# lhotse-speech/lhotse

Measured on AMD Instinct MI355X. Metric: cuts/sec (10 s @16 kHz -> 80-dim log-mel fbank), higher is better.
Workload: dtype f32

## Files before the change

### lhotse_amd/csrc/fft_common.hpp

```cpp
#pragma once
#include "common.hpp"

namespace hipfeat {

typedef float v2 __attribute__((ext_vector_type(2)));
typedef float f32x4 __attribute__((ext_vector_type(4)));

template <int CTRL>
__device__ __forceinline__ float dpp_mov(float v) {
  return __builtin_bit_cast(float, __builtin_amdgcn_update_dpp(0, __builtin_bit_cast(int, v), CTRL, 0xF, 0xF, true));
}
__device__ __forceinline__ float dpp_shr1_keep(float keep, float v) {
  return __builtin_bit_cast(float, __builtin_amdgcn_update_dpp(__builtin_bit_cast(int, keep), __builtin_bit_cast(int, v), 0x111, 0xF, 0xF, false));
}
constexpr int DPP_QUAD(int a, int b, int c, int d) { return a | (b << 2) | (c << 4) | (d << 6); }
constexpr int DPP_ROW_SHR1 = 0x111;
constexpr int DPP_ROW_ROR1 = 0x121;
constexpr int DPP_ROW_MIRROR = 0x140;
constexpr int DPP_ROW_HALF_MIRROR = 0x141;

__device__ __forceinline__ float row16_sum(float v) {
  v += dpp_mov<DPP_QUAD(1, 0, 3, 2)>(v);
  v += dpp_mov<DPP_QUAD(2, 3, 0, 1)>(v);
  v += dpp_mov<DPP_ROW_HALF_MIRROR>(v);
// ... 75 lines not shown
    const v2 d = hi ? x[n] - x[n + 16] : x[n];
    if (n == 0) o[n] = d;
    else if (n == 8) o[n] = rot_mi(d);
    else o[n] = cmulc(d, v2{C[n], -S[n]}, v2{S[n], C[n]});
  }
  fft16(e, E);
  fft16(o, O);
#pragma unroll
  for (int k = 0; k < 16; ++k) {
    X[2 * k] = E[k];
    X[2 * k + 1] = O[k];
  }
}

__device__ __forceinline__ void fft8(const v2* x, v2* X) {
  constexpr float R2 = 0.70710678118654752f;
  v2 e[4], o[4];
  {
    const v2 s0 = x[0] + x[4], s1 = x[0] - x[4], s2 = x[2] + x[6], u3 = swap2(x[2] - x[6]);
    e[0] = s0 + s2, e[2] = s0 - s2, e[1] = u3 * HF_CJ + s1, e[3] = u3 * HF_NCJ + s1;
  }
  {
    const v2 s0 = x[1] + x[5], s1 = x[1] - x[5], s2 = x[3] + x[7], u3 = swap2(x[3] - x[7]);
    o[0] = s0 + s2, o[2] = s0 - s2, o[1] = u3 * HF_CJ + s1, o[3] = u3 * HF_NCJ + s1;
  }
  o[1] = cmulc(o[1], v2{R2, -R2}, v2{R2, R2});
  o[2] = rot_mi(o[2]);
  o[3] = cmulc(o[3], v2{-R2, -R2}, v2{R2, -R2});
#pragma unroll
  for (int k = 0; k < 4; ++k) {
    X[k] = e[k] + o[k];
    X[k + 4] = e[k] - o[k];
  }
}

__device__ __forceinline__ void mel4_reduce_floor(const f32x4 acc, float m4, float m8, float floor_, float (&v)[4]) {
  float v0 = acc[0], v1 = acc[1], v2_ = acc[2], v3 = acc[3];
  asm volatile(
      "s_nop 7\n\t"
      "v_fmac_f32_dpp %0, %0, %4 row_shr:4 row_mask:0xf bank_mask:0xf bound_ctrl:1\n\t"
      "v_fmac_f32_dpp %1, %1, %4 row_shr:4 row_mask:0xf bank_mask:0xf bound_ctrl:1\n\t"
      "v_fmac_f32_dpp %2, %2, %4 row_shr:4 row_mask:0xf bank_mask:0xf bound_ctrl:1\n\t"
      "v_fmac_f32_dpp %3, %3, %4 row_shr:4 row_mask:0xf bank_mask:0xf bound_ctrl:1\n\t"
      "v_fmac_f32_dpp %0, %0, %5 row_shr:8 row_mask:0xf bank_mask:0xf bound_ctrl:1\n\t"
      "v_fmac_f32_dpp %1, %1, %5 row_shr:8 row_mask:0xf bank_mask:0xf bound_ctrl:1\n\t"
      "v_fmac_f32_dpp %2, %2, %5 row_shr:8 row_mask:0xf bank_mask:0xf bound_ctrl:1\n\t"
      "v_fmac_f32_dpp %3, %3, %5 row_shr:8 row_mask:0xf bank_mask:0xf bound_ctrl:1\n\t"
      "v_max_f32 %0, %0, %6\n\tv_max_f32 %1, %1, %6\n\tv_max_f32 %2, %2, %6\n\tv_max_f32 %3, %3, %6"
      : "+v"(v0), "+v"(v1), "+v"(v2_), "+v"(v3)
      : "v"(m4), "v"(m8), "v"(floor_));
  v[0] = v0, v[1] = v1, v[2] = v2_, v[3] = v3;
}
template <int ROWS>
__device__ __forceinline__ void mel4_store(float* o, int64_t stride, int nf, const float* v) {
  if (nf >= ROWS) {
#pragma unroll
    for (int i = 0; i < ROWS; ++i) o[i * stride] = v[i];
  } else {
#pragma unroll
    for (int i = 0; i < ROWS - 1; ++i)
      if (i < nf) o[i * stride] = v[i];
  }
}
template <int ROWS>
__device__ __forceinline__ void mel4_store_saddr(float* row0, unsigned col, int64_t stride, int nf, const float* v) {
  const unsigned off = col * 4u;
#pragma unroll
  for (int i = 0; i < ROWS; ++i) {
    if (i < nf) {
      const float* base = row0 + i * stride;
      asm volatile("global_store_dword %0, %1, %2" : : "v"(off), "v"(v[i]), "s"(base) : "memory");
    }
  }
}

__device__ __forceinline__ float fast_log(float x) {
#ifdef HIPFEAT_ACCURATE_LOG
  return logf(x);
#else
  return __builtin_amdgcn_logf(x) * 0.69314718055994531f;
#endif
}

}
```

### lhotse_amd/csrc/hipfeat.hip

```cpp
#include "../../include/hipfeat.h"

#include <hip/hip_runtime.h>

#include <algorithm>
#include <atomic>
#include <cmath>
#include <cstdarg>
#include <cstdio>
#include <cstring>
#include <map>
#include <mutex>
#include <new>
#include <string>
#include <vector>

#include "common.hpp"
#include "kernel_generic.hpp"
#include "fft512_common.hpp"
#include "kernel_fft512b.hpp"
#include "kernel_fft512c.hpp"
#include "kernel_fft1024c.hpp"
#include "kernel_fft2048c.hpp"
#include "plan_tables.hpp"
#include "kernel_resample.hpp"
// ... 5 lines not shown
#include "kernel_level.hpp"
#include "kernel_sinc.hpp"
#include "kernel_specaug.hpp"
#include "kernel_whisper2.hpp"
#include "kernel_whisper3.hpp"
#include "layout_rounds.hpp"
#include "kernel_fft256.hpp"
#include "kernel_fft256c.hpp"
#include "kernel_wave.hpp"
#include "host_bulk.hpp"

using namespace hipfeat;

static thread_local char g_err[512] = "";

static inline const char* route_env(const char* name) { return getenv(name); }
#ifdef HIPFEAT_EXPERIMENTS
static inline const char* exp_env(const char* name) { return getenv(name); }
#else
static inline const char* exp_env(const char*) { return nullptr; }
#endif

static hipfeat_status fail(hipfeat_status st, const char* fmt, ...) {
  va_list ap;
  va_start(ap, fmt);
  vsnprintf(g_err, sizeof(g_err), fmt, ap);
  va_end(ap);
  return st;
}

#define HIP_TRY(expr)                                                                          \
  do {                                                                                         \
    hipError_t e_ = (expr);                                                                    \
    if (e_ != hipSuccess)                                                                      \
      return fail(HIPFEAT_ERR_HIP, "%s failed: %s (%s:%d)", #expr, hipGetErrorName(e_), __FILE__, __LINE__); \
  } while (0)

struct DeviceGuard {
  int prev = -1;
  bool ok = true;
  explicit DeviceGuard(int dev) {
    if (hipGetDevice(&prev) != hipSuccess) prev = -1;
    if (prev != dev) ok = (hipSetDevice(dev) == hipSuccess);
  }
  ~DeviceGuard() {
    int cur = -1;
    if (prev >= 0 && hipGetDevice(&cur) == hipSuccess && cur != prev) (void)hipSetDevice(prev);
  }
};

struct StagingSlot {
  void* h = nullptr;
  void* d = nullptr;
  size_t cap = 0;
  hipEvent_t ev = nullptr;
  bool busy = false;
};

enum class Route {
  Generic,
  Fft512b,
  Fft256b,
  Wave,
  Whisper2,
  Fft512c,
  Fft1024c,
  Whisper3,
  Fft2048c,
  Fft256c,
};

struct hipfeat_plan {
  hipfeat_config cfg{};
  int device = 0;
  int feature_dim = 0;
  int K = 0, H = 0, log2H = 0;
  bool pow2 = false;
  int npad_left = 0;
  std::string kernel_name = "generic";
  int blocks_per_cu = 0;
  Route route = Route::Generic;
  const void* fn = nullptr;
  const void* fn_flat = nullptr;
  int block = 0;
  size_t lds = 0;
  float* d_window = nullptr;
  float2* d_tw = nullptr;
  float* d_mel = nullptr;
  int2* d_mel_range = nullptr;
  float* d_dct = nullptr;
  float* d_lifter = nullptr;
  int fpb = 8;
  int span = 0, off_z = 0, off_p = 0, off_tw = 0, off_stat = 0, off_mel = 0;
  float* d_mel_a4 = nullptr;
  float* d_dct_consts = nullptr;
  int lm_stride = 0, dct_groups = 0, dct_floats = 0;
  int tiles_per_block = 4;
  int xs_floats = 0;
  int const_floats = 0;
  float* d_lds_consts = nullptr;
  float* d_mel_a = nullptr;
  WaveWork* d_work = nullptr;
  float* d_c_shared = nullptr;
  int c_shared_floats = 0, c_wtab_off = 0, c_ltab_off = 0, c_xs_floats = 0;
  int fpb_unit = 0, c_rounds_max = 0;
  int w_nsets = 0, w_steps[kWMaxSets] = {}, w_step0[kWMaxSets] = {};
  float* d_x_twp = nullptr;
  int x_waves = 0, x_tws_off = 0, x_tw32_off = 0;
  float* d_mel_t = nullptr;
  int wave_blob_floats = 0;
  bool wave_dct_in_lds = false;
  float* d_wh2_cs = nullptr;
  float* d_wh2_tw = nullptr;
  float* d_wh2_mel = nullptr;
  int32_t* d_wh2_sched = nullptr;
  mutable std::mutex mu;
  mutable StagingSlot slots[4];
  mutable int next_slot = 0;
  mutable float* d_scratch_wave = nullptr;
  mutable size_t scratch_wave_cap = 0;
  mutable float* d_scratch_out = nullptr;
  mutable size_t scratch_out_cap = 0;
};

struct hipfeat_layout {
  int device = 0;
  int64_t batch = 0;
  int64_t total_frames = 0;
  int64_t total_blocks = 0;
  int64_t out_row_stride = 0;
  int uniform_bpc = 0;
  int fpb = 0, fpb_unit = 0;
  CutDesc* d_cuts = nullptr;
  bool owns = true;
  std::vector<int64_t> num_frames;
  std::vector<int32_t> block_cut;
  bool flat = false;
  int64_t total_quads = 0;
  unsigned char* d_norm = nullptr;
  int norm_slots = 0;
  mutable std::atomic<unsigned> norm_next{0};
};
constexpr int kNormSlots = 4;
static size_t norm_slot_bytes(const hipfeat_layout* lay) { return (2 * (size_t)lay->total_blocks + (size_t)lay->batch) * 4; }

extern "C" HIPFEAT_API int32_t hipfeat_abi_version(void) { return HIPFEAT_ABI_VERSION; }
extern "C" HIPFEAT_API const char* hipfeat_last_error(void) { return g_err; }

extern "C" HIPFEAT_API hipfeat_status hipfeat_device_count(int32_t* count) {
  if (!count) return fail(HIPFEAT_ERR_INVALID, "count is NULL");
  int n = 0;
  hipError_t e = hipGetDeviceCount(&n);
  if (e != hipSuccess) {
    *count = 0;
    return fail(HIPFEAT_ERR_HIP, "hipGetDeviceCount failed: %s", hipGetErrorName(e));
  }
  *count = n;
  return HIPFEAT_OK;
}

extern "C" HIPFEAT_API int64_t hipfeat_num_frames(int64_t num_samples, int32_t frame_length, int32_t frame_shift,
                                      int32_t snip_edges) {
  if (frame_shift <= 0 || frame_length <= 0 || num_samples < 0) return 0;
  if (snip_edges) return num_samples < frame_length ? 0 : 1 + (num_samples - frame_length) / frame_shift;
  return (num_samples + frame_shift / 2) / frame_shift;
}
// ... 66 lines not shown
}

#ifdef HIPFEAT_LDS_POISON
static void set_lds_poison(size_t bytes) {
  const int n = (int)(bytes / sizeof(float));
  (void)hipMemcpyToSymbol(HIP_SYMBOL(hipfeat::g_lds_poison_floats), &n, sizeof(n));
}
#else
static inline void set_lds_poison(size_t) {}
#endif

static hipError_t ensure_dynamic_lds(const void* fn, size_t bytes) {
  static std::mutex mu;
  static std::map<std::pair<const void*, int>, size_t> high;
  int dev = 0;
  (void)hipGetDevice(&dev);
  std::lock_guard<std::mutex> lk(mu);
  size_t& cur = high[{fn, dev}];
  if (bytes <= cur) return hipSuccess;
  hipError_t e = hipFuncSetAttribute(fn, hipFuncAttributeMaxDynamicSharedMemorySize, (int)bytes);
  if (e == hipSuccess) cur = bytes;
  return e;
}

static hipfeat_status claim(hipfeat_plan* p, Route route, const void* fn, int block, size_t lds) {
  hipError_t e = ensure_dynamic_lds(fn, lds);
  if (e != hipSuccess) return fail(HIPFEAT_ERR_HIP, "hipFuncSetAttribute(dynamic LDS = %zu B) failed: %s", lds, hipGetErrorName(e));
  int nb = 0;
  if (hipOccupancyMaxActiveBlocksPerMultiprocessor(&nb, fn, block, lds) == hipSuccess) p->blocks_per_cu = nb;
  p->route = route;
  p->fn = fn;
  p->block = block;
  p->lds = lds;
  return HIPFEAT_OK;
}

static hipfeat_status claim_wave_auto(hipfeat_plan* p, Route route, const void* fn, const WaveAutoTables& t, int frames, int rounds, int rounds_max,
                                      const std::string& head) {
  hipfeat_status st;
  if ((st = upload(&p->d_c_shared, t.image.data(), t.image.size())) != HIPFEAT_OK) return st;
  if (!t.dct.empty() && (st = upload(&p->d_dct_consts, t.dct.data(), t.dct.size())) != HIPFEAT_OK) return st;
  if (!t.twp.empty() && (st = upload(&p->d_x_twp, t.twp.data(), t.twp.size())) != HIPFEAT_OK) return st;
  p->c_shared_floats = t.shared_floats;
  p->c_wtab_off = t.wtab_off;
  p->c_ltab_off = t.ltab_off;
  p->c_xs_floats = t.xs_floats;
  p->x_tws_off = t.tws_off;
  p->x_tw32_off = t.tw32_off;
  p->w_nsets = t.w_nsets;
  std::copy(t.w_steps, t.w_steps + 4, p->w_steps);
  std::copy(t.w_step0, t.w_step0 + 4, p->w_step0);
  p->fpb_unit = t.waves * frames;
  p->fpb = p->fpb_unit * rounds;
  p->c_rounds_max = rounds_max;
  if ((st = claim(p, route, fn, 64 * t.waves, t.lds)) != HIPFEAT_OK) return st;
  p->kernel_name = head + strf(" lds=%zuB blocks/CU=%d mel4=%dx%d", t.lds, p->blocks_per_cu, t.sch_nsets, t.sch_steps);
  return HIPFEAT_OK;
}

static hipfeat_status claim_tile(hipfeat_plan* p, Route route, const void* fn, const TileTables& t, int tile_frames, const char* kernel) {
  const hipfeat_config& c = p->cfg;
  const bool mfcc = c.kind == HIPFEAT_MFCC, spec = c.kind == HIPFEAT_SPECTROGRAM || c.kind == HIPFEAT_LOG_SPECTROGRAM;
  hipfeat_status st;
  if ((st = upload(&p->d_lds_consts, t.consts.data(), t.consts.size())) != HIPFEAT_OK) return st;
  if (route == Route::Fft512b && (st = upload(&p->d_mel_a, t.mel_a.data(), t.mel_a.size())) != HIPFEAT_OK) return st;
  if ((st = upload(&p->d_work, t.work, 4)) != HIPFEAT_OK) return st;
  if ((st = upload(&p->d_mel_a4, t.mel_a4.data(), t.mel_a4.size())) != HIPFEAT_OK) return st;
  if (mfcc && (st = upload(&p->d_dct_consts, t.dct.data(), t.dct.size())) != HIPFEAT_OK) return st;
  p->tiles_per_block = 16;
  p->fpb = tile_frames * p->tiles_per_block;
  p->const_floats = (int)t.consts.size();
  p->xs_floats = t.xs_floats;
  p->lm_stride = t.lm_stride;
  p->dct_groups = t.dct_groups;
  p->dct_floats = (int)t.dct.size();
  if ((st = claim(p, route, fn, 256, t.lds)) != HIPFEAT_OK) return st;
  p->kernel_name = strf("%s<%d,%d> %s lds=%zuB blocks/CU=%d", kernel, t.nrows, mfcc ? 1 : (spec ? 2 : 0), mfcc ? "mfcc" : (spec ? "spectrogram" : "fbank"), t.lds,
                        p->blocks_per_cu);
  return HIPFEAT_OK;
}

static bool fft512c_has_flat(int nrows, int N) { return nrows == 13 && N >= 384; }

template <int MODE>
static const void* fft512c_pick(int nrows, int N, bool flat) {
  if (flat && fft512c_has_flat(nrows, N)) return entry<fft512c_kernel<13, 12, MODE, true>>();
  if (nrows == 10) return entry<fft512c_kernel<10, 0, MODE>>();
  if (nrows == 13 && N >= 384) return entry<fft512c_kernel<13, 12, MODE>>();
  if (nrows == 13) return entry<fft512c_kernel<13, 0, MODE>>();
  return entry<fft512c_kernel<16, 0, MODE>>();
}
static const void* fft512c_dispatch(int mode, int nrows, int N, bool flat) {
  return mode == 0 ? fft512c_pick<0>(nrows, N, flat)
                   : (mode == 1 ? fft512c_pick<1>(nrows, N, flat) : (mode == 2 ? fft512c_pick<2>(nrows, N, flat) : fft512c_pick<3>(nrows, N, flat)));
}

static hipfeat_status setup_fft512c(hipfeat_plan* p, const PlanInputs& in, int nrows) {
  const bool mfcc = p->cfg.kind == HIPFEAT_MFCC;
  if (mfcc && (in.M > 4 * kCDctChunks || in.C > 64 || !in.dct)) return HIPFEAT_OK;
  const WaveAutoTables t = build_fft512c_tables(in, nrows, {kCPRowStride, kCMaxSets, kCMaxSteps, kCWaves, kCRegion}, kCDctChunks, kCDctChunksSmall);
  if (!t.fits || t.lds > 80 * 1024 || (t.xs_floats >> 8) > 6) return HIPFEAT_OK;
  hipfeat_status st = claim_wave_auto(p, Route::Fft512c, fft512c_dispatch(t.mode, nrows, in.N, false), t, 4, 8, 16,
                                      strf("fft512c_kernel<%d> %s", nrows, mfcc ? "mfcc" : "fbank"));
  if (st == HIPFEAT_OK && fft512c_has_flat(nrows, in.N)) {
    p->fn_flat = fft512c_dispatch(t.mode, nrows, in.N, true);
    hipError_t e = ensure_dynamic_lds(p->fn_flat, t.lds);
    if (e != hipSuccess) return fail(HIPFEAT_ERR_HIP, "hipFuncSetAttribute(dynamic LDS = %zu B) failed: %s", t.lds, hipGetErrorName(e));
  }
  return st;
}

static hipfeat_status setup_fft512(hipfeat_plan* p, const PlanInputs& in) {
  const hipfeat_config& c = p->cfg;
  const char* force = route_env("HIPFEAT_FORCE_GENERIC");
  if (force && force[0] == '1') return HIPFEAT_OK;
  const bool mfcc = c.kind == HIPFEAT_MFCC;
  const bool spec = c.kind == HIPFEAT_SPECTROGRAM || c.kind == HIPFEAT_LOG_SPECTROGRAM;
  if (c.kind > HIPFEAT_MFCC || c.fft_length != 512 || (in.shift & 1) || in.N < 32 || c.use_energy || (!spec && c.use_fft_mag))
    return HIPFEAT_OK;
  if (mfcc && (in.M > 8 * kMaxDctGroups || in.C > 64)) return HIPFEAT_OK;
  const int need = (in.N + 31) / 32;
  const int nrows = need <= 10 ? 10 : (need <= 13 ? 13 : 16);
  if ((in.M + 15) / 16 > 8) return HIPFEAT_OK;

  if (!spec) {
    const char* var = route_env("HIPFEAT_FFT512_VARIANT");
    if (!(var && var[0] == 'b')) {
      hipfeat_status stc = setup_fft512c(p, in, nrows);
      if (stc != HIPFEAT_OK || p->route == Route::Fft512c) return stc;
    }
  }
  const TileTables t = build_tile_tables(in, nrows, {16, kPRowStride, kMaxGroups0, kMaxGroups1, kTileFrames, kBWaveRegion, false});
  if (!t.fits || t.lds > 160 * 1024) return HIPFEAT_OK;
  const void* fn;
  if (mfcc)
    fn = nrows == 10 ? entry<fft512b_kernel<10, 1>>() : (nrows == 13 ? entry<fft512b_kernel<13, 1>>() : entry<fft512b_kernel<16, 1>>());
  else if (spec)
    fn = nrows == 10 ? entry<fft512b_kernel<10, 2>>() : (nrows == 13 ? entry<fft512b_kernel<13, 2>>() : entry<fft512b_kernel<16, 2>>());
  else
    fn = nrows == 10 ? entry<fft512b_kernel<10, 0>>() : (nrows == 13 ? entry<fft512b_kernel<13, 0>>() : entry<fft512b_kernel<16, 0>>());
  return claim_tile(p, Route::Fft512b, fn, t, kTileFrames, "fft512b_kernel");
}

static hipfeat_status setup_fft1024c(hipfeat_plan* p, const PlanInputs& in) {
  const hipfeat_config& c = p->cfg;
  const int N = in.N, shift = in.shift;
  const bool librosa = c.kind == HIPFEAT_LIBROSA_FBANK;
  if ((c.kind != HIPFEAT_FBANK && !librosa) || c.fft_length != 1024 || (shift & 1) || N < 32 * 17 || c.use_energy ||
      (c.use_fft_mag && !librosa) || route_env("HIPFEAT_FORCE_GENERIC") || route_env("HIPFEAT_NO_WAVE_AUTONOMOUS"))
    return HIPFEAT_OK;
  const int need = (N + 31) / 32;
  const int nrows = need <= 20 ? 20 : (need <= 26 ? 26 : 32);
  static const int kFixedSteps[5][3] = {{0, 0, 0}, {24, 16, 8}, {24, 16, 8}, {24, 24, 8}, {16, 16, 8}};
  int want = 0;
  if (route_env("HIPFEAT_NO_FIXED_SCHEDULE")) want = 0;
  else if (nrows == 32) want = !c.remove_dc_offset && c.preemph_coeff == 0.0f ? 4 : 0;
  else if (!librosa && !c.use_fft_mag && in.M == 80 && !c.snip_edges)
    want = N == 600 && shift == 240 ? 1 : (N == 800 && shift == 320 ? 2 : (N == 551 && shift == 220 ? 3 : 0));
  const WaveAutoTables t = build_fft1024c_tables(in, nrows, {kWPRowStride, kWMaxSets, kWMaxSteps, kWWaves, kWRegion}, kWSplitSteps, kWWavesFixed, want ? kFixedSteps[want] : nullptr);
  if (!t.fits || t.lds > 160 * 1024 || (t.xs_floats >> 8) > 10) return HIPFEAT_OK;
  const int fixed = t.fixed ? want : 0;
  const void* fn = fixed == 1 ? entry<fft1024c_kernel<20, 24, 16, 8>>()
                   : fixed == 2 ? entry<fft1024c_kernel<26, 24, 16, 8>>()
                   : fixed == 3 ? entry<fft1024c_kernel<20, 24, 24, 8>>()
                   : fixed == 4 ? entry<fft1024c_kernel<32, 16, 16, 8, true>>()
                   : nrows == 20 ? entry<fft1024c_kernel<20>>() : (nrows == 26 ? entry<fft1024c_kernel<26>>() : entry<fft1024c_kernel<32>>());
  return claim_wave_auto(p, Route::Fft1024c, fn, t, 4, 8, 32, strf("fft1024c_kernel<%d> fbank%s waves=%d", nrows, fixed ? " fixed-schedule" : "", t.waves));
}

static hipfeat_status setup_fft256c(hipfeat_plan* p, const PlanInputs& in, int nrows) {
  const WaveAutoTables t = build_fft256c_tables(in, nrows, {kDPRowStride, kDSets, kDSteps, kDWaves, kDRegion});
  if (!t.fits || t.lds > 80 * 1024 || (t.xs_floats >> 8) > 6) return HIPFEAT_OK;
  const void* fn = nrows == 13 ? (in.N >= 192 ? entry<fft256c_kernel<13, 12>>() : entry<fft256c_kernel<13, 0>>()) : entry<fft256c_kernel<16, 0>>();
  return claim_wave_auto(p, Route::Fft256c, fn, t, 8, 4, 16, strf("fft256c_kernel<%d> fbank", nrows));
}

static hipfeat_status setup_fft256(hipfeat_plan* p, const PlanInputs& in) {
  const hipfeat_config& c = p->cfg;
  const bool mfcc = c.kind == HIPFEAT_MFCC;
  const bool spec = c.kind == HIPFEAT_SPECTROGRAM || c.kind == HIPFEAT_LOG_SPECTROGRAM;
  if (c.kind > HIPFEAT_MFCC || c.fft_length != 256 || (in.shift & 1) || in.N < 16 || c.use_energy || (!spec && c.use_fft_mag) ||
      route_env("HIPFEAT_FORCE_GENERIC"))
    return HIPFEAT_OK;
  if (mfcc && (in.M > 8 * kMaxDctGroups || in.C > 64)) return HIPFEAT_OK;
  const int nrows = (in.N + 15) / 16 <= 13 ? 13 : 16;
  if ((in.M + 15) / 16 > 8) return HIPFEAT_OK;
  if (!mfcc && !spec) {
    const char* var = route_env("HIPFEAT_FFT256_VARIANT");
    if (!(var && var[0] == 'b') && !route_env("HIPFEAT_NO_WAVE_AUTONOMOUS")) {
// ... 516 lines not shown
      w2.out = d_out;
      w2.cuts = lay->d_cuts;
      w2.window = plan->d_window;
      w2.cs = plan->d_wh2_cs;
      w2.tw = plan->d_wh2_tw;
      w2.mel_a = plan->d_wh2_mel;
      w2.out_stride = lay->out_row_stride;
      w2.num_cuts = (int32_t)lay->batch;
      w2.uniform_bpc = lay->uniform_bpc;
      w2.M = c.num_filters;
      w2.mel_floor = c.mel_floor;
      w2.sched = plan->d_wh2_sched;
      arg = &w2;
      break;
    case Route::Whisper3:
      fill_wave_autonomous(w3, plan, lay, d_wave, d_out);
      w3.cs = plan->d_wh2_cs;
      w3.total_blocks = (int32_t)lay->total_blocks;
      if (lay->d_norm) {
        unsigned char* slot = lay->d_norm + (size_t)(lay->norm_next.fetch_add(1u) % (unsigned)lay->norm_slots) * norm_slot_bytes(lay);
        w3.wg_stat = reinterpret_cast<float*>(slot);
        w3.cut_done = reinterpret_cast<uint32_t*>(slot + 2 * (size_t)lay->total_blocks * sizeof(float));
      }
      arg = &w3;
      break;
    case Route::Fft512c:
      cp.dct_tab = plan->d_dct_consts;
      cp.C = c.num_ceps;
      cp.total_quads = (int32_t)lay->total_quads;
      [[fallthrough]];
    case Route::Fft256c:
      fill_wave_autonomous(cp, plan, lay, d_wave, d_out);
      fill_frames(cp, plan);
      arg = &cp;
      break;
    case Route::Fft1024c:
      fill_wave_autonomous(kp, plan, lay, d_wave, d_out);
      fill_frames(kp, plan);
      kp.nsets = plan->w_nsets;
      for (int s2 = 0; s2 < kWMaxSets; ++s2) kp.steps[s2] = plan->w_steps[s2], kp.step0[s2] = plan->w_step0[s2];
      arg = &kp;
      break;
    case Route::Fft2048c:
      fill_wave_autonomous(xp, plan, lay, d_wave, d_out);
      fill_frames(xp, plan);
      xp.twp = plan->d_x_twp;
      xp.waves = plan->x_waves;
      xp.tws_off = plan->x_tws_off;
      xp.tw32_off = plan->x_tw32_off;
      xp.nsets = plan->w_nsets;
      for (int s2 = 0; s2 < kXMaxSets; ++s2) xp.steps[s2] = plan->w_steps[s2], xp.step0[s2] = plan->w_step0[s2];
      arg = &xp;
      break;
    case Route::Fft512b:
    case Route::Fft256b:
      bp.wave = d_wave;
      bp.out = d_out;
      bp.cuts = lay->d_cuts;
      bp.lds_consts = plan->d_lds_consts;
      bp.mel_a = plan->d_mel_a4;
      bp.work = plan->d_work;
      bp.out_stride = lay->out_row_stride;
      bp.num_cuts = (int32_t)lay->batch;
      bp.uniform_bpc = lay->uniform_bpc;
      bp.tiles_per_block = plan->tiles_per_block;
      bp.N = c.frame_length;
      bp.shift = c.frame_shift;
      bp.npad_left = plan->npad_left;
      bp.M = c.num_filters;
      bp.flags = (c.remove_dc_offset ? F_REMOVE_DC : 0) | (c.use_fft_mag ? F_FFT_MAG : 0) | (c.kind == HIPFEAT_LOG_SPECTROGRAM ? F_LOG_SPEC : 0);
      bp.log_offset = c.log_offset;
      bp.preemph = c.preemph_coeff;
      bp.mel_floor = c.mel_floor;
      bp.xs_floats = plan->xs_floats;
      bp.const_floats = plan->const_floats;
      bp.dct_consts = plan->d_dct_consts;
      bp.C = c.num_ceps;
      bp.lm_stride = plan->lm_stride;
      bp.dct_groups = plan->dct_groups;
      bp.dct_floats = plan->dct_floats;
      arg = &bp;
      break;
  }
  const void* fn = lay->flat && plan->fn_flat ? plan->fn_flat : plan->fn;
  void* args[] = {arg};
  DeviceGuard g(plan->device);
  set_lds_poison(plan->lds);
  (void)hipLaunchKernel(fn, dim3((unsigned)lay->total_blocks), dim3(plan->block), args, plan->lds, stream);
  HIP_TRY(hipGetLastError());
  if (whisper && !(plan->route == Route::Whisper3 && lay->d_norm)) {
    hipLaunchKernelGGL(whisper_norm_kernel, dim3((unsigned)lay->batch), dim3(1024), 0, stream, lay->d_cuts, d_out, lay->out_row_stride,
                       (int32_t)c.num_filters, (int32_t)c.frame_shift);
    HIP_TRY(hipGetLastError());
  }
  return HIPFEAT_OK;
}

extern "C" HIPFEAT_API hipfeat_status hipfeat_extract_layout(const hipfeat_plan* plan, const hipfeat_layout* layout,
                                                 const float* d_wave, float* d_out, void* stream) {
  if (!plan || !layout) return fail(HIPFEAT_ERR_INVALID, "plan/layout is NULL");
  return launch(plan, layout, d_wave, d_out, (hipStream_t)stream);
}

__global__ __launch_bounds__(256) void fill_padding_kernel(const CutDesc* __restrict__ cuts, float* __restrict__ out, int64_t row_stride,
                                                           int32_t rows_per_cut, int32_t feature_dim, float value) {
  const CutDesc cd = cuts[blockIdx.y];
  const int64_t n = (int64_t)(rows_per_cut - cd.num_frames) * feature_dim;
  float* __restrict__ base = out + (cd.out_row + cd.num_frames) * row_stride;
  for (int64_t i = (int64_t)blockIdx.x * 256 + threadIdx.x; i < n; i += (int64_t)gridDim.x * 256) {
    const int64_t r = i / feature_dim;
    base[r * row_stride + (i - r * feature_dim)] = value;
  }
}

__global__ __launch_bounds__(256) void pcm16_to_float_kernel(const int16_t* __restrict__ in, float* __restrict__ out, int64_t n) {
  const int64_t n8 = n >> 3;
  const bool aligned = ((reinterpret_cast<uintptr_t>(in) & 15) == 0) && ((reinterpret_cast<uintptr_t>(out) & 15) == 0);
  constexpr float k = 1.0f / 32768.0f;
  if (aligned) {
    for (int64_t i = (int64_t)blockIdx.x * 256 + threadIdx.x; i < n8; i += (int64_t)gridDim.x * 256) {
      const int4 v = reinterpret_cast<const int4*>(in)[i];
      const int w[4] = {v.x, v.y, v.z, v.w};
      float4 a, b;
      a.x = (float)(int16_t)(w[0] & 0xffff) * k; a.y = (float)(w[0] >> 16) * k;
      a.z = (float)(int16_t)(w[1] & 0xffff) * k; a.w = (float)(w[1] >> 16) * k;
      b.x = (float)(int16_t)(w[2] & 0xffff) * k; b.y = (float)(w[2] >> 16) * k;
      b.z = (float)(int16_t)(w[3] & 0xffff) * k; b.w = (float)(w[3] >> 16) * k;
      reinterpret_cast<float4*>(out)[2 * i] = a;
      reinterpret_cast<float4*>(out)[2 * i + 1] = b;
    }
    for (int64_t i = (n8 << 3) + (int64_t)blockIdx.x * 256 + threadIdx.x; i < n; i += (int64_t)gridDim.x * 256) out[i] = (float)in[i] * k;
  } else {
    for (int64_t i = (int64_t)blockIdx.x * 256 + threadIdx.x; i < n; i += (int64_t)gridDim.x * 256) out[i] = (float)in[i] * k;
  }
}

extern "C" HIPFEAT_API hipfeat_status hipfeat_pcm16_to_float(const int16_t* d_pcm, float* d_wave, int64_t num_samples, void* stream) {
  if (num_samples < 0 || (num_samples > 0 && (!d_pcm || !d_wave))) return fail(HIPFEAT_ERR_INVALID, "bad pcm16 arguments");
  if (num_samples == 0) return HIPFEAT_OK;
  const int64_t blocks = std::min<int64_t>((num_samples / 8 + 255) / 256 + 1, 256 * 32);
  hipLaunchKernelGGL(pcm16_to_float_kernel, dim3((unsigned)blocks), dim3(256), 0, (hipStream_t)stream, d_pcm, d_wave, num_samples);
  hipError_t e = hipGetLastError();
  if (e != hipSuccess) return fail(HIPFEAT_ERR_HIP, "pcm16 launch failed: %s", hipGetErrorName(e));
  return HIPFEAT_OK;
}

__global__ __launch_bounds__(256) void float_to_half_kernel(const float* __restrict__ in, uint16_t* __restrict__ out, int64_t n) {
  const int64_t n8 = n >> 3;
  const bool aligned = ((reinterpret_cast<uintptr_t>(in) & 15) == 0) && ((reinterpret_cast<uintptr_t>(out) & 15) == 0);
  auto cvt = [](float x) -> unsigned { return (unsigned)__builtin_bit_cast(unsigned short, (_Float16)x); };
  if (aligned) {
    for (int64_t i = (int64_t)blockIdx.x * 256 + threadIdx.x; i < n8; i += (int64_t)gridDim.x * 256) {
      const float4 a = reinterpret_cast<const float4*>(in)[2 * i], b = reinterpret_cast<const float4*>(in)[2 * i + 1];
      uint4 o;
      o.x = cvt(a.x) | (cvt(a.y) << 16);
      o.y = cvt(a.z) | (cvt(a.w) << 16);
      o.z = cvt(b.x) | (cvt(b.y) << 16);
      o.w = cvt(b.z) | (cvt(b.w) << 16);
      reinterpret_cast<uint4*>(out)[i] = o;
    }
    for (int64_t i = (n8 << 3) + (int64_t)blockIdx.x * 256 + threadIdx.x; i < n; i += (int64_t)gridDim.x * 256) out[i] = (uint16_t)cvt(in[i]);
  } else {
    for (int64_t i = (int64_t)blockIdx.x * 256 + threadIdx.x; i < n; i += (int64_t)gridDim.x * 256) out[i] = (uint16_t)cvt(in[i]);
  }
}

extern "C" HIPFEAT_API hipfeat_status hipfeat_float_to_half(const float* d_in, uint16_t* d_out, int64_t n, void* stream) {
// ... 1698 lines not shown
```

### lhotse_amd/csrc/kernel_fft512c.hpp

```cpp
#pragma once
#include "common.hpp"
#include "fft_common.hpp"

namespace hipfeat {

constexpr int kCExRowStride = 34;
constexpr int kCExFrameStride = 8 * kCExRowStride + 16;
constexpr int kCPRowStride = 272;
constexpr int kCRegion = 4 * kCExFrameStride + 16;
constexpr int kCMaxSets = 2;
constexpr int kCMaxSteps = 16;
constexpr int kCWaves = 8;
constexpr int kCLmStride = 48;
constexpr int kCDctChunks = 10;
constexpr int kCDctChunksSmall = 6;

struct Fft512cParams {
  const float* wave;
  float* out;
  const CutDesc* cuts;
  const float* shared_consts;
  int64_t out_stride;
  int32_t num_cuts, uniform_bpc;
  int32_t frames_per_block, rounds;
  int32_t N, shift, npad_left, M, flags;
  float preemph, mel_floor;
  int32_t shared_floats;
  int32_t wtab_off, ltab_off;
  int32_t xs_floats;
  const float* dct_tab;
  int32_t C;
  int32_t total_quads;
};

#ifdef HIPFEAT_PHASE_TIMERS
#define HFC_T(i) { const unsigned long long tt_ = __builtin_readcyclecounter(); hfc_acc[i] += tt_ - hfc_last; hfc_last = tt_; }
#else
#define HFC_T(i)
#endif
#define HFC_SEP() asm volatile("")
__device__ __forceinline__ int mul24(int a, int b) { return (int)__umul24((unsigned)a, (unsigned)b); }

__device__ __forceinline__ void exchange_halves(unsigned wr, unsigned rd, unsigned long long hi_lanes, v2 (&lo)[8], const v2 (&hi)[8],
                                                v2 (&up)[8]) {
  static_assert(kCExRowStride == 34, "the row offsets below are 17 rr (in 8-byte units)");
  unsigned long long saved;
  asm volatile(
      "ds_write2_b64 %[wr], %[l0], %[l1] offset1:17\n\t"
      "ds_write2_b64 %[wr], %[l2], %[l3] offset0:34 offset1:51\n\t"
      "ds_write2_b64 %[wr], %[l4], %[l5] offset0:68 offset1:85\n\t"
      "ds_write2_b64 %[wr], %[l6], %[l7] offset0:102 offset1:119\n\t"
      "ds_read_b64 %[l0], %[rd]\n\t"
      "ds_read_b64 %[l1], %[rd] offset:8\n\t"
      "ds_read_b64 %[l2], %[rd] offset:16\n\t"
      "ds_read_b64 %[l3], %[rd] offset:24\n\t"
      "ds_read_b64 %[l4], %[rd] offset:32\n\t"
      "ds_read_b64 %[l5], %[rd] offset:40\n\t"
      "ds_read_b64 %[l6], %[rd] offset:48\n\t"
      "ds_read_b64 %[l7], %[rd] offset:56\n\t"
      "ds_read_b64 %[u0], %[rd] offset:64\n\t"
      "ds_read_b64 %[u1], %[rd] offset:72\n\t"
      "ds_read_b64 %[u2], %[rd] offset:80\n\t"
      "ds_read_b64 %[u3], %[rd] offset:88\n\t"
      "ds_read_b64 %[u4], %[rd] offset:96\n\t"
      "ds_read_b64 %[u5], %[rd] offset:104\n\t"
      "ds_read_b64 %[u6], %[rd] offset:112\n\t"
      "ds_read_b64 %[u7], %[rd] offset:120\n\t"
      "ds_write2_b64 %[wr], %[h0], %[h1] offset1:17\n\t"
      "ds_write2_b64 %[wr], %[h2], %[h3] offset0:34 offset1:51\n\t"
      "ds_write2_b64 %[wr], %[h4], %[h5] offset0:68 offset1:85\n\t"
      "ds_write2_b64 %[wr], %[h6], %[h7] offset0:102 offset1:119\n\t"
      "s_and_saveexec_b64 %[sv], %[hm]\n\t"
      "ds_read_b64 %[l0], %[rd]\n\t"
      "ds_read_b64 %[l1], %[rd] offset:8\n\t"
      "ds_read_b64 %[l2], %[rd] offset:16\n\t"
      "ds_read_b64 %[l3], %[rd] offset:24\n\t"
      "ds_read_b64 %[l4], %[rd] offset:32\n\t"
      "ds_read_b64 %[l5], %[rd] offset:40\n\t"
      "ds_read_b64 %[l6], %[rd] offset:48\n\t"
      "ds_read_b64 %[l7], %[rd] offset:56\n\t"
      "ds_read_b64 %[u0], %[rd] offset:64\n\t"
      "ds_read_b64 %[u1], %[rd] offset:72\n\t"
      "ds_read_b64 %[u2], %[rd] offset:80\n\t"
      "ds_read_b64 %[u3], %[rd] offset:88\n\t"
      "ds_read_b64 %[u4], %[rd] offset:96\n\t"
      "ds_read_b64 %[u5], %[rd] offset:104\n\t"
      "ds_read_b64 %[u6], %[rd] offset:112\n\t"
      "ds_read_b64 %[u7], %[rd] offset:120\n\t"
      "s_mov_b64 exec, %[sv]\n\t"
      "s_waitcnt lgkmcnt(0)"
      : [l0] "+&v"(lo[0]), [l1] "+&v"(lo[1]), [l2] "+&v"(lo[2]), [l3] "+&v"(lo[3]), [l4] "+&v"(lo[4]), [l5] "+&v"(lo[5]),
        [l6] "+&v"(lo[6]), [l7] "+&v"(lo[7]), [u0] "=&v"(up[0]), [u1] "=&v"(up[1]), [u2] "=&v"(up[2]), [u3] "=&v"(up[3]),
        [u4] "=&v"(up[4]), [u5] "=&v"(up[5]), [u6] "=&v"(up[6]), [u7] "=&v"(up[7]), [sv] "=&s"(saved)
      : [h0] "v"(hi[0]), [h1] "v"(hi[1]), [h2] "v"(hi[2]), [h3] "v"(hi[3]), [h4] "v"(hi[4]), [h5] "v"(hi[5]), [h6] "v"(hi[6]),
        [h7] "v"(hi[7]), [wr] "v"(wr), [rd] "v"(rd), [hm] "s"(hi_lanes)
      : "memory", "scc");
}

template <int NROWS, int NFULL, int MODE, bool FLAT = false>
__global__ __launch_bounds__(64 * kCWaves, 4) void fft512c_kernel(const Fft512cParams p) {
  extern __shared__ __attribute__((aligned(16))) float smem[];
  HF_POISON_LDS(smem);
  const v2* cwin = reinterpret_cast<const v2*>(smem);
  const v2* ctwp = cwin + NROWS * 16;
  const v2* ctws = ctwp + 256;
  const float* wtab = smem + p.wtab_off;
  const float* ltab = smem + p.ltab_off;

  const int tid = threadIdx.x;
  const int lane = tid & 63;
  const int wv = __builtin_amdgcn_readfirstlane(tid >> 6);

  const int blk = blockIdx.x;
  int cut, fb;
  if (FLAT) {
    cut = __builtin_amdgcn_readfirstlane(block_cut_map(p.cuts, p.num_cuts)[blk]);
    fb = 0;
  } else if (p.uniform_bpc > 0) {
    cut = blk / p.uniform_bpc;
    fb = blk - cut * p.uniform_bpc;
  } else {
    cut = p.uniform_bpc < 0 ? block_cut_map(p.cuts, p.num_cuts)[blk] : find_cut(p.cuts, p.num_cuts, blk);
    fb = blk - p.cuts[cut].first_block;
  }
  CutDesc cd = FLAT ? load_cut_uniform(p.cuts + cut) : p.cuts[cut];
  const int N = p.N, shift = p.shift;

  for (int i = tid; i < p.shared_floats; i += 64 * kCWaves) smem[i] = p.shared_consts[i];
  float* xs = smem + p.shared_floats + wv * (p.xs_floats + kCRegion);
  float* myreg = xs + p.xs_floats;
  const bool dc = (p.flags & F_REMOVE_DC) != 0;
  const float inv_n = 1.0f / (float)N;
  const float c = p.preemph;

  auto stage_span = [&](const CutDesc& cd, int f0, unsigned lane4) {
    const float* __restrict__ w = p.wave + cd.wave_off;
    const int64_t j0 = (int64_t)f0 * shift - p.npad_left;
    if (j0 >= 0 && j0 + p.xs_floats <= cd.num_samples) {
      const char* src = reinterpret_cast<const char*>(w + j0);
      const int nfull = p.xs_floats >> 8;
#pragma unroll
      for (int ch = 0; ch < 6; ++ch) {
        if (ch < nfull)
          __builtin_amdgcn_global_load_lds((const __attribute__((address_space(1))) void*)(src + ((unsigned)ch * 1024u + 4u * lane4)),
                                           (__attribute__((address_space(3))) void*)(xs + ch * 256), 16, 0, 0);
      }
      if ((unsigned)nfull * 256u + lane4 < (unsigned)p.xs_floats)
        __builtin_amdgcn_global_load_lds((const __attribute__((address_space(1))) void*)(src + ((unsigned)nfull * 1024u + 4u * lane4)),
                                         (__attribute__((address_space(3))) void*)(xs + nfull * 256), 16, 0, 0);
    } else {
      for (int i = (int)(lane4 >> 2); i < p.xs_floats; i += 64) xs[i] = load_sample(w, j0 + i, cd.num_samples, cd.padded_len);
    }
  };

  const int first_frame = fb * p.frames_per_block + 4 * wv;
  int quad = 0, next_first = 0, f0_flat = 0;
  int cut_n = 0, quad_n = 0, next_first_n = 0, f0_n = 0;
  CutDesc cd_n = cd;
  auto advance = [&](int q, int& c, CutDesc& d, int& nfirst) {
    while (c + 1 < p.num_cuts && q >= nfirst) {
      ++c;
      d = load_cut_uniform(p.cuts + c);
      nfirst = c + 1 < p.num_cuts ? __builtin_amdgcn_readfirstlane(p.cuts[c + 1].first_block) : p.total_quads;
    }
  };
  if (FLAT) {
    quad = blk * (p.frames_per_block >> 2) + wv;
    next_first = cut + 1 < p.num_cuts ? __builtin_amdgcn_readfirstlane(p.cuts[cut + 1].first_block) : p.total_quads;
    advance(quad, cut, cd, next_first);
    f0_flat = 4 * (quad - cd.first_block);
    cut_n = cut, cd_n = cd, next_first_n = next_first, quad_n = quad + kCWaves;
    advance(quad_n, cut_n, cd_n, next_first_n);
    f0_n = 4 * (quad_n - cd_n.first_block);
  }
  __syncthreads();
  if (FLAT ? quad < p.total_quads : first_frame < cd.num_frames) stage_span(cd, FLAT ? f0_flat : first_frame, (unsigned)lane * 4u);

  constexpr bool kMfcc = MODE == 2 || MODE == 3;
  constexpr int DCH = MODE == 3 ? kCDctChunksSmall : kCDctChunks;
#ifdef HIPFEAT_ABL_MFCC_TWS
  constexpr bool kTwsExp = MODE == 2 && NROWS <= 13;
#else
  constexpr bool kTwsExp = false;
#endif
  constexpr int DREG = kTwsExp ? 6 : (MODE == 2 && NROWS > 13) ? 5 : DCH;
  constexpr bool kDctLate = DREG < DCH;
  constexpr bool kRegTw = !kMfcc && NROWS <= 13;
  constexpr bool kRegTws = kRegTw || (MODE == 3 && NROWS <= 13) || kTwsExp;
  v2 twpreg[kRegTw ? 16 : 1], twsreg[kRegTws ? 8 : 1];
  if (kRegTw) {
#pragma unroll
    for (int k1 = 1; k1 < 16; ++k1) twpreg[k1] = ctwp[k1 * 16 + (lane & 15)];
  }
  if (kRegTws) {
#pragma unroll
    for (int k2 = 0; k2 < 8; ++k2) twsreg[k2] = ctws[k2 * 16 + (lane & 15)];
  }
  f32x4 dw[kMfcc ? DREG : 1];
  float lift = 1.0f;
  if (kMfcc) {
#pragma unroll
    for (int c4 = 0; c4 < DREG; ++c4) dw[c4] = *reinterpret_cast<const f32x4*>(p.dct_tab + (c4 * 64 + lane) * 4);
    lift = p.dct_tab[DCH * 256 + lane];
  }
#ifdef HIPFEAT_PHASE_TIMERS
  unsigned long long hfc_acc[8] = {0, 0, 0, 0, 0, 0, 0, 0}, hfc_last = __builtin_readcyclecounter();
#endif
  for (int r = 0; r < p.rounds; ++r) {
    const int f0 = FLAT ? f0_flat : first_frame + 4 * kCWaves * r;
    if (FLAT ? quad >= p.total_quads : f0 >= cd.num_frames) break;
    const int nf = min(4, cd.num_frames - f0);

    if (r == 0)
    __builtin_amdgcn_s_waitcnt(0x0F70);
    HFC_T(0);
    int lane_o = lane;
    asm volatile("" : "+v"(lane_o));
    const int q = lane_o & 15, g = lane_o >> 4;

    f32x4 lt4[2];
    v2 Z[16];
    {
      const float* x = xs + mul24(g, shift) + 2 * q;
      v2 z[16];
      v2 win[NROWS];
      v2 sum2 = {0.f, 0.f};
#pragma unroll
      for (int n1 = 0; n1 < NROWS; ++n1) {
        z[n1] = *reinterpret_cast<const v2*>(x + 32 * n1);
        HFC_SEP();
      }
      float pv[NROWS];
// ... 108 lines not shown
        v2 tw[4];
        if (kRegTws) {
#pragma unroll
          for (int rr = 0; rr < 4; ++rr) tw[rr] = twsreg[4 * h + rr];
        } else {
#pragma unroll
          for (int rr = 0; rr < 4; ++rr) {
            tw[rr] = ctws[(4 * h + rr) * 16 + q];
            HFC_SEP();
          }
        }
#pragma unroll
        for (int rr = 0; rr < 4; ++rr) {
          const int k2 = 4 * h + rr;
          const v2 m = v2{t1[2 * k2], t1[2 * k2 + 1]};
          const v2 sp = m * HF_CJ + Z[k2];
          const v2 dm = m * HF_NCJ + Z[k2];
          const v2 tt = cmul2(dm, tw[rr]);
          v2 re2, im2, pw;
          asm("v_pk_fma_f32 %0, %1, %2, %3 op_sel:[0,0,0] op_sel_hi:[0,1,0]" : "=v"(re2) : "v"(tt), "v"(HF_CJ), "v"(sp));
          asm("v_pk_fma_f32 %0, %1, %2, %3 op_sel:[1,0,1] op_sel_hi:[1,1,1]" : "=v"(im2) : "v"(tt), "v"(HF_CJ), "v"(sp));
          pw = re2 * re2;
          pw = im2 * im2 + pw;
#ifdef HIPFEAT_ABL_NO_POWER
          asm volatile("" : : "v"(pw.x), "v"(pw.y));
#else
          pown[16 * k2] = pw.x;
          ppar[16 * (15 - k2)] = pw.y;
#endif
        }
      }
      if (q == 0) prow[128] = 4.f * (Z[8].x * Z[8].x + Z[8].y * Z[8].y);
    }
    HFC_T(4);
    __builtin_amdgcn_fence(__ATOMIC_RELEASE, "wavefront");
    __builtin_amdgcn_wave_barrier();
    __builtin_amdgcn_fence(__ATOMIC_ACQUIRE, "wavefront");

    __builtin_amdgcn_s_waitcnt(0x0F70);
    f32x4 dwx[kDctLate ? DCH - DREG : 1];
    if (kDctLate) {
#pragma unroll
      for (int c4 = DREG; c4 < DCH; ++c4) dwx[c4 - DREG] = *reinterpret_cast<const f32x4*>(p.dct_tab + (c4 * 64 + lane_o) * 4);
    }
    float* orow = p.out + (cd.out_row + f0) * p.out_stride;
    constexpr int S = MODE == 0 ? kCMaxSets : 1, T = MODE == 0 ? kCMaxSteps : 2 * kCMaxSteps;
    int lt_poff[S], lt_col[S];
    float lt_m4[S], lt_m8[S];
#pragma unroll
    for (int s = 0; s < S; ++s) {
      const float poff_f = lt4[s][0], col_f = lt4[s][1];
      lt_poff[s] = __builtin_bit_cast(int, poff_f);
      lt_col[s] = __builtin_bit_cast(int, col_f);
      lt_m4[s] = lt4[s][2];
      lt_m8[s] = lt4[s][3];
    }
    f32x4 av[S][T / 4], bv[S][T / 4];
#pragma unroll
    for (int s = 0; s < S; ++s) {
      const float* pa = myreg + lt_poff[s];
      const float* wb = wtab + s * (T * 64) + 4 * lane_o;
#pragma unroll
      for (int c4 = 0; c4 < T / 4; ++c4) {
#if defined(HIPFEAT_ABL_NO_MELOPS) || defined(HIPFEAT_ABL_NO_MEL_A)
        av[s][c4] = f32x4{1.f, 2.f, 3.f, 4.f} * __builtin_bit_cast(float, lane_o);
#else
        av[s][c4] = *reinterpret_cast<const f32x4*>(pa + 4 * c4);
#endif
#if defined(HIPFEAT_ABL_NO_MELOPS) || defined(HIPFEAT_ABL_NO_MEL_B)
        bv[s][c4] = f32x4{1.f, 2.f, 3.f, 4.f} * __builtin_bit_cast(float, lane_o + c4);
#else
        bv[s][c4] = *reinterpret_cast<const f32x4*>(wb + c4 * 256);
#endif
      }
    }
    HFC_T(5);
    float lm[4];
    {
      f32x4 acc[2] = {{0.f, 0.f, 0.f, 0.f}, {0.f, 0.f, 0.f, 0.f}};
#pragma unroll
      for (int c4 = 0; c4 < (S * T) / 8; ++c4) {
#pragma unroll
        for (int i = 0; i < 4; ++i) {
          if (MODE == 0) {
            acc[0] = __builtin_amdgcn_mfma_f32_4x4x1f32(av[0][c4][i], bv[0][c4][i], acc[0], 0, 0, 0);
            acc[1] = __builtin_amdgcn_mfma_f32_4x4x1f32(av[S - 1][c4][i], bv[S - 1][c4][i], acc[1], 0, 0, 0);
          } else {
            acc[0] = __builtin_amdgcn_mfma_f32_4x4x1f32(av[0][2 * c4][i], bv[0][2 * c4][i], acc[0], 0, 0, 0);
            acc[1] = __builtin_amdgcn_mfma_f32_4x4x1f32(av[0][2 * c4 + 1][i], bv[0][2 * c4 + 1][i], acc[1], 0, 0, 0);
          }
        }
      }
      if (MODE != 0) acc[0] += acc[1];
      float val[S][4];
#pragma unroll
      for (int s = 0; s < S; ++s) {
        mel4_reduce_floor(acc[s], lt_m4[s], lt_m8[s], p.mel_floor, val[s]);
#pragma unroll
        for (int i = 0; i < 4; ++i) val[s][i] = fast_log(val[s][i]);
      }
#pragma unroll
      for (int s = 0; s < S; ++s) {
        const int col = lt_col[s];
        if (kMfcc) {
#pragma unroll
          for (int i = 0; i < 4; ++i) lm[i] = val[s][i];
        } else if (col < p.M) {
          mel4_store_saddr<4>(orow, (unsigned)col, p.out_stride, nf, val[s]);
        }
      }
    }
    if (kMfcc) {
      float* lmrow = myreg;
      const int col = lt_col[0];
      if (col < p.M) {
#pragma unroll
        for (int i = 0; i < 4; ++i) lmrow[i * kCLmStride + col] = lm[i];
      }
      __builtin_amdgcn_fence(__ATOMIC_RELEASE, "wavefront");
      __builtin_amdgcn_wave_barrier();
      __builtin_amdgcn_fence(__ATOMIC_ACQUIRE, "wavefront");
      f32x4 al[DCH];
#pragma unroll
      for (int c4 = 0; c4 < DCH; ++c4) al[c4] = *reinterpret_cast<const f32x4*>(lmrow + (lane_o & 3) * kCLmStride + 4 * c4);
      f32x4 d0 = {0.f, 0.f, 0.f, 0.f}, d1 = {0.f, 0.f, 0.f, 0.f};
#pragma unroll
      for (int c4 = 0; c4 < DCH; ++c4) {
#pragma unroll
        for (int i = 0; i < 4; i += 2) {
          const f32x4 w4 = (kDctLate && c4 >= DREG) ? dwx[c4 >= DREG ? c4 - DREG : 0] : dw[c4 < DREG ? c4 : 0];
          d0 = __builtin_amdgcn_mfma_f32_4x4x1f32(al[c4][i], w4[i], d0, 0, 0, 0);
          d1 = __builtin_amdgcn_mfma_f32_4x4x1f32(al[c4][i + 1], w4[i + 1], d1, 0, 0, 0);
        }
      }
      d0 += d1;
      if (lane_o < p.C) {
#pragma unroll
        for (int i = 0; i < 4; ++i)
          if (i < nf) orow[i * p.out_stride + lane_o] = d0[i] * lift;
      }
    }
    HFC_T(6);
#ifdef HIPFEAT_PHASE_TIMERS
    hfc_acc[7] += 1;
#endif
    if (FLAT) {
      quad = quad_n, cut = cut_n, cd = cd_n, next_first = next_first_n, f0_flat = f0_n;
      quad_n += kCWaves;
      advance(quad_n, cut_n, cd_n, next_first_n);
      f0_n = 4 * (quad_n - cd_n.first_block);
    }
  }
#ifdef HIPFEAT_PHASE_TIMERS
  if (lane == 0 && g_phase_buf) {
    unsigned long long* o = g_phase_buf + ((size_t)blockIdx.x * kCWaves + wv) * 8;
    for (int i = 0; i < 8; ++i) o[i] = hfc_acc[i];
  }
#endif
}

}
```

Measured before the change: 3.035 million.

## Transpose mel MFMA to emit 16-byte row stores and branchless span staging

Swaps the MFMA operand order in the log-mel epilogue so each lane holds four consecutive mel columns of one frame. The result is then written with a single global_store_dwordx4 instead of four strided scalar stores, and the log is applied only on lanes that store. Variants for very large output strides fall back to the old path, and a ten-second wave load is now done with fixed asm global_load_lds pieces masked by exec rather than per-chunk branches. The change adds more kernel instantiations, inline asm that depends on a 24-bit stride multiply, and a tighter cap on span size.

```diff
diff --git a/lhotse_amd/csrc/fft_common.hpp b/lhotse_amd/csrc/fft_common.hpp
--- a/lhotse_amd/csrc/fft_common.hpp
+++ b/lhotse_amd/csrc/fft_common.hpp
@@ -181,4 +181,18 @@
 #endif
 }
 
+constexpr int64_t kMel4WideMaxStride = 1 << 22;
+__device__ __forceinline__ void mel4_store_wide(float* row0, int lane, unsigned col0, int M, int stride, int nf, const float (&v)[4]) {
+  const int fr = lane & 3;
+  if (col0 < (unsigned)M && fr < nf) {
+    f32x4 o;
+#pragma unroll
+    for (int i = 0; i < 4; ++i) o[i] = fast_log(v[i]);
+    unsigned rowoff;
+    asm("v_mul_u32_u24 %0, %1, %2" : "=v"(rowoff) : "v"(fr), "s"(stride));
+    const unsigned off = (rowoff + col0) << 2;
+    asm volatile("global_store_dwordx4 %0, %1, %2" : : "v"(off), "v"(o), "s"(row0) : "memory");
+  }
 }
+
+}
diff --git a/lhotse_amd/csrc/hipfeat.hip b/lhotse_amd/csrc/hipfeat.hip
--- a/lhotse_amd/csrc/hipfeat.hip
+++ b/lhotse_amd/csrc/hipfeat.hip
@@ -111,6 +111,8 @@
   Route route = Route::Generic;
   const void* fn = nullptr;
   const void* fn_flat = nullptr;
+  const void* fn_far = nullptr;
+  const void* fn_flat_far = nullptr;
   int block = 0;
   size_t lds = 0;
   float* d_window = nullptr;
@@ -343,15 +345,16 @@
 
 static bool fft512c_has_flat(int nrows, int N) { return nrows == 13 && N >= 384; }
 
-template <int MODE>
+template <int MODE, bool WIDE = false>
 static const void* fft512c_pick(int nrows, int N, bool flat) {
-  if (flat && fft512c_has_flat(nrows, N)) return entry<fft512c_kernel<13, 12, MODE, true>>();
-  if (nrows == 10) return entry<fft512c_kernel<10, 0, MODE>>();
-  if (nrows == 13 && N >= 384) return entry<fft512c_kernel<13, 12, MODE>>();
-  if (nrows == 13) return entry<fft512c_kernel<13, 0, MODE>>();
-  return entry<fft512c_kernel<16, 0, MODE>>();
-}
-static const void* fft512c_dispatch(int mode, int nrows, int N, bool flat) {
+  if (flat && fft512c_has_flat(nrows, N)) return entry<fft512c_kernel<13, 12, MODE, true, WIDE>>();
+  if (nrows == 10) return entry<fft512c_kernel<10, 0, MODE, false, WIDE>>();
+  if (nrows == 13 && N >= 384) return entry<fft512c_kernel<13, 12, MODE, false, WIDE>>();
+  if (nrows == 13) return entry<fft512c_kernel<13, 0, MODE, false, WIDE>>();
+  return entry<fft512c_kernel<16, 0, MODE, false, WIDE>>();
+}
+static const void* fft512c_dispatch(int mode, int nrows, int N, bool flat, bool wide) {
+  if (wide && mode <= 1) return mode == 0 ? fft512c_pick<0, true>(nrows, N, flat) : fft512c_pick<1, true>(nrows, N, flat);
   return mode == 0 ? fft512c_pick<0>(nrows, N, flat)
                    : (mode == 1 ? fft512c_pick<1>(nrows, N, flat) : (mode == 2 ? fft512c_pick<2>(nrows, N, flat) : fft512c_pick<3>(nrows, N, flat)));
 }
@@ -360,12 +363,17 @@
   const bool mfcc = p->cfg.kind == HIPFEAT_MFCC;
   if (mfcc && (in.M > 4 * kCDctChunks || in.C > 64 || !in.dct)) return HIPFEAT_OK;
   const WaveAutoTables t = build_fft512c_tables(in, nrows, {kCPRowStride, kCMaxSets, kCMaxSteps, kCWaves, kCRegion}, kCDctChunks, kCDctChunksSmall);
-  if (!t.fits || t.lds > 80 * 1024 || (t.xs_floats >> 8) > 6) return HIPFEAT_OK;
-  hipfeat_status st = claim_wave_auto(p, Route::Fft512c, fft512c_dispatch(t.mode, nrows, in.N, false), t, 4, 8, 16,
+  if (!t.fits || t.lds > 80 * 1024 || t.xs_floats > 256 * kCSpanPieces) return HIPFEAT_OK;
+  const bool wide = !mfcc && t.mode <= 1 && in.M % 4 == 0 && !route_env("HIPFEAT_NO_WIDE_STORE");
+  hipfeat_status st = claim_wave_auto(p, Route::Fft512c, fft512c_dispatch(t.mode, nrows, in.N, false, wide), t, 4, 8, 16,
                                       strf("fft512c_kernel<%d> %s", nrows, mfcc ? "mfcc" : "fbank"));
-  if (st == HIPFEAT_OK && fft512c_has_flat(nrows, in.N)) {
-    p->fn_flat = fft512c_dispatch(t.mode, nrows, in.N, true);
-    hipError_t e = ensure_dynamic_lds(p->fn_flat, t.lds);
+  if (st == HIPFEAT_OK && wide) p->kernel_name += " store=16B";
+  const void** more[3] = {&p->fn_flat, &p->fn_far, &p->fn_flat_far};
+  for (int i = 0; st == HIPFEAT_OK && i < 3; ++i) {
+    const bool flat = i != 1, far = i != 0;
+    if ((flat && !fft512c_has_flat(nrows, in.N)) || (far && !wide)) continue;
+    *more[i] = fft512c_dispatch(t.mode, nrows, in.N, flat, wide && !far);
+    hipError_t e = ensure_dynamic_lds(*more[i], t.lds);
     if (e != hipSuccess) return fail(HIPFEAT_ERR_HIP, "hipFuncSetAttribute(dynamic LDS = %zu B) failed: %s", t.lds, hipGetErrorName(e));
   }
   return st;
@@ -1048,7 +1056,8 @@
       arg = &bp;
       break;
   }
-  const void* fn = lay->flat && plan->fn_flat ? plan->fn_flat : plan->fn;
+  const bool far = plan->fn_far && lay->out_row_stride >= kMel4WideMaxStride;
+  const void* fn = lay->flat && plan->fn_flat ? (far ? plan->fn_flat_far : plan->fn_flat) : (far ? plan->fn_far : plan->fn);
   void* args[] = {arg};
   DeviceGuard g(plan->device);
   set_lds_poison(plan->lds);
diff --git a/lhotse_amd/csrc/kernel_fft512c.hpp b/lhotse_amd/csrc/kernel_fft512c.hpp
--- a/lhotse_amd/csrc/kernel_fft512c.hpp
+++ b/lhotse_amd/csrc/kernel_fft512c.hpp
@@ -97,7 +97,34 @@
       : "memory", "scc");
 }
 
-template <int NROWS, int NFULL, int MODE, bool FLAT = false>
+constexpr int kCSpanPieces = 4;
+__device__ __forceinline__ void span_pieces(const char* src, unsigned lds, unsigned lane_bytes, int span_bytes) {
+  static_assert(kCSpanPieces == 4, "the immediate offset reaches 4095");
+  unsigned long long saved;
+  int rem;
+  asm volatile(
+      "v_sub_u32 %[rem], %[sb], %[lb]\n\t"
+      "s_mov_b32 m0, %[lds]\n\t"
+      "s_mov_b64 %[sv], exec\n\t"
+      "v_cmp_lt_i32 vcc, 0, %[rem]\n\t"
+      "s_and_b64 exec, %[sv], vcc\n\t"
+      "global_load_lds_dwordx4 %[lb], %[src]\n\t"
+      "v_cmp_lt_i32 vcc, 0x400, %[rem]\n\t"
+      "s_and_b64 exec, %[sv], vcc\n\t"
+      "global_load_lds_dwordx4 %[lb], %[src] offset:1024\n\t"
+      "v_cmp_lt_i32 vcc, 0x800, %[rem]\n\t"
+      "s_and_b64 exec, %[sv], vcc\n\t"
+      "global_load_lds_dwordx4 %[lb], %[src] offset:2048\n\t"
+      "v_cmp_lt_i32 vcc, 0xc00, %[rem]\n\t"
+      "s_and_b64 exec, %[sv], vcc\n\t"
+      "global_load_lds_dwordx4 %[lb], %[src] offset:3072\n\t"
+      "s_mov_b64 exec, %[sv]"
+      : [rem] "=&v"(rem), [sv] "=&s"(saved)
+      : [sb] "s"(span_bytes), [lb] "v"(lane_bytes), [lds] "s"(lds), [src] "s"(src)
+      : "memory", "vcc", "scc", "m0");
+}
+
+template <int NROWS, int NFULL, int MODE, bool FLAT = false, bool WIDE = false>
 __global__ __launch_bounds__(64 * kCWaves, 4) void fft512c_kernel(const Fft512cParams p) {
   extern __shared__ __attribute__((aligned(16))) float smem[];
   HF_POISON_LDS(smem);
@@ -129,6 +156,7 @@
   for (int i = tid; i < p.shared_floats; i += 64 * kCWaves) smem[i] = p.shared_consts[i];
   float* xs = smem + p.shared_floats + wv * (p.xs_floats + kCRegion);
   float* myreg = xs + p.xs_floats;
+  static_assert(!WIDE || MODE == 0 || MODE == 1, "the 16-byte store is the log-mel epilogue's");
   const bool dc = (p.flags & F_REMOVE_DC) != 0;
   const float inv_n = 1.0f / (float)N;
   const float c = p.preemph;
@@ -136,8 +164,12 @@
   auto stage_span = [&](const CutDesc& cd, int f0, unsigned lane4) {
     const float* __restrict__ w = p.wave + cd.wave_off;
     const int64_t j0 = (int64_t)f0 * shift - p.npad_left;
-    if (j0 >= 0 && j0 + p.xs_floats <= cd.num_samples) {
+    if (__builtin_expect(j0 >= 0 && j0 + p.xs_floats <= cd.num_samples, 1)) {
       const char* src = reinterpret_cast<const char*>(w + j0);
+#ifndef HIPFEAT_ABL_SPAN_BRANCHES
+      typedef __attribute__((address_space(3))) float lds_float;
+      span_pieces(src, (unsigned)(size_t)(lds_float*)xs, 4u * lane4, 4 * p.xs_floats);
+#else
       const int nfull = p.xs_floats >> 8;
 #pragma unroll
       for (int ch = 0; ch < 6; ++ch) {
@@ -148,6 +180,7 @@
       if ((unsigned)nfull * 256u + lane4 < (unsigned)p.xs_floats)
         __builtin_amdgcn_global_load_lds((const __attribute__((address_space(1))) void*)(src + ((unsigned)nfull * 1024u + 4u * lane4)),
                                          (__attribute__((address_space(3))) void*)(xs + nfull * 256), 16, 0, 0);
+#endif
     } else {
       for (int i = (int)(lane4 >> 2); i < p.xs_floats; i += 64) xs[i] = load_sample(w, j0 + i, cd.num_samples, cd.padded_len);
     }
@@ -422,7 +455,13 @@
       for (int c4 = 0; c4 < (S * T) / 8; ++c4) {
 #pragma unroll
         for (int i = 0; i < 4; ++i) {
-          if (MODE == 0) {
+          if (MODE == 0 && WIDE) {
+            acc[0] = __builtin_amdgcn_mfma_f32_4x4x1f32(bv[0][c4][i], av[0][c4][i], acc[0], 0, 0, 0);
+            acc[1] = __builtin_amdgcn_mfma_f32_4x4x1f32(bv[S - 1][c4][i], av[S - 1][c4][i], acc[1], 0, 0, 0);
+          } else if (WIDE) {
+            acc[0] = __builtin_amdgcn_mfma_f32_4x4x1f32(bv[0][2 * c4][i], av[0][2 * c4][i], acc[0], 0, 0, 0);
+            acc[1] = __builtin_amdgcn_mfma_f32_4x4x1f32(bv[0][2 * c4 + 1][i], av[0][2 * c4 + 1][i], acc[1], 0, 0, 0);
+          } else if (MODE == 0) {
             acc[0] = __builtin_amdgcn_mfma_f32_4x4x1f32(av[0][c4][i], bv[0][c4][i], acc[0], 0, 0, 0);
             acc[1] = __builtin_amdgcn_mfma_f32_4x4x1f32(av[S - 1][c4][i], bv[S - 1][c4][i], acc[1], 0, 0, 0);
           } else {
@@ -436,13 +475,18 @@
 #pragma unroll
       for (int s = 0; s < S; ++s) {
         mel4_reduce_floor(acc[s], lt_m4[s], lt_m8[s], p.mel_floor, val[s]);
-#pragma unroll
-        for (int i = 0; i < 4; ++i) val[s][i] = fast_log(val[s][i]);
+        if (!WIDE) {
+#pragma unroll
+          for (int i = 0; i < 4; ++i) val[s][i] = fast_log(val[s][i]);
+        }
       }
 #pragma unroll
       for (int s = 0; s < S; ++s) {
         const int col = lt_col[s];
-        if (kMfcc) {
+        if (WIDE) {
+          const int col0 = __builtin_amdgcn_update_dpp(0, col, DPP_QUAD(0, 0, 0, 0), 0xF, 0xF, true);
+          mel4_store_wide(orow, lane_o, (unsigned)col0, p.M, (int)p.out_stride, nf, val[s]);
+        } else if (kMfcc) {
 #pragma unroll
           for (int i = 0; i < 4; ++i) lm[i] = val[s][i];
         } else if (col < p.M) {
```

Measured after the change: 3.082 million (median of 6 runs). 1.02x the previous value.
